# HiLab-git/WSL4MIS

Hardware: AMD Instinct MI355X
Metric: training slices/sec (256x256, bs64, unet_cct pCE+GatedCRF) (higher is better)
Workload: dtype f32; 1 GPU; unet_cct pce_gatedcrf r=5, 256x256x1 4-class synthetic scribble slices, batch 64/GPU, SGD+poly LR; global_batch=64, parallelism=dp1, crf_radius=5, conv_precision=f32

## Files before the change

include/wsl_hip.h:

```cpp
#ifndef WSL_HIP_H
#define WSL_HIP_H
#include <stddef.h>
#include <stdint.h>

#ifdef __cplusplus
extern "C" {
#endif

#define WSL_OK 0
#define WSL_EINVAL (-1)
#define WSL_EUNSUPPORTED (-2)
#define WSL_EHIP (-3)
#define WSL_EWORKSPACE (-4)

#define WSL_LEAKY_SLOPE 0.01f

int wsl_version(void);
const char* wsl_last_error(void);
const char* wsl_build_info(void);

#define WSL_PROF_FAMILIES 20
typedef struct WslProfRow {
  char name[48];
  int64_t calls;
// ... 43 lines not shown
                          int64_t* num_batches_tracked, float* mean, float* invstd, float* scale, float* shift,
                          void* stream);
int wsl_bn_eval_affine(const float* gamma, const float* beta, const float* running_mean, const float* running_var,
                       float eps, int C, float* scale, float* shift, void* stream);
int wsl_src_materialize(const WslSrc* s, float* out, int64_t out_bs, int N, int H, int W, void* stream);
int wsl_pool2_fwd(const WslSrc* s, float* out, int N, int H, int W, void* stream);

int wsl_feat_grad_combine(const WslSrc* f, const float* ga, int64_t ga_bs, const float* gb, int64_t gb_bs,
                          const float* gb_cmask, const float* gp, float* g, int N, int H, int W, void* stream);

int wsl_bnact_bwd(const float* g, int64_t g_bs, const float* y, const float* mean, const float* invstd,
                  const float* gamma, const float* beta, const uint8_t* emask, float emask_scale, float* dy,
                  float* dgamma, float* dbeta, int N, int C, int H, int W, void* ws, size_t ws_bytes, void* stream);
size_t wsl_bnact_bwd_ws_bytes(int N, int C, int H, int W);

int wsl_conv2d_dgrad_bn(const WslSrc* dy, const float* w, float* g, int64_t g_bs, int N, int H, int W, int Co, int ks,
                        int wmode, const float* bn_y, const float* bn_st, const uint8_t* bn_emask, float bn_emask_scale,
                        float* bn_part, int* fused, void* stream);
int wsl_feat_grad_combine_blocks(int N, int H, int W);
int wsl_feat_grad_combine_bn(const WslSrc* f, const float* ga, int64_t ga_bs, const float* gb, int64_t gb_bs,
                             const float* gb_cmask, const float* gp, float* g, int N, int H, int W, const float* bn_mean,
                             const float* bn_invstd, float* bn_part, void* stream);
int wsl_bnact_bwd_finish(const float* g, int64_t g_bs, const float* y, const float* mean, const float* invstd,
                         const float* gamma, const float* beta, const uint8_t* emask, float emask_scale, float* dy,
                         float* dgamma, float* dbeta, int N, int C, int H, int W, const float* part, int nblk,
                         int channel_major, void* ws, size_t ws_bytes, void* stream);
int wsl_conv2d_dgrad_bn_d(const WslSrc* dy, const float* w, float* g, int64_t g_bs, int N, int H, int W, int Co, int ks,
                          int wmode, const float* bn_y, const float* bn_st, const uint8_t* bn_emask, float bn_emask_scale,
                          float* bn_part, int* fused, void* stream);
int wsl_bnact_bwd_finish_d_amax(const float* dz, int64_t dz_bs, const float* y, const float* mean, const float* invstd,
                                const float* gamma, const float* beta, float* dy, float* dgamma, float* dbeta, int N, int C, int H,
                                int W, const float* part, int nblk, int channel_major, void* ws, size_t ws_bytes, uint32_t* dy_amax,
                                void* stream);

#define WSL_SP_ACT_EXP 4
#define WSL_SP_AMAX_SLOTS 64
int wsl_sp_conv2d_ok(const WslSrc* a, const WslSrc* b, const float* y, int64_t y_bs, int N, int H, int W, int Co, int ks);
size_t wsl_sp_weight_image_bytes(int Co, int Ci);
int wsl_sp_pack_weights(const float* w, void* image, uint32_t* w_amax, int Co, int Ci, int dgrad, void* stream);
int wsl_sp_conv2d_fwd(const WslSrc* a, const WslSrc* b, const void* image, const uint32_t* w_amax, const uint32_t* in_amax,
                      const float* bias, float* y, int64_t y_bs, int N, int H, int W, int Co, float* stat_part, float* stat_cnt,
                      void* stream);
int wsl_sp_conv2d_stat_blocks(int N, int H, int W, int Ci, int Co);
int wsl_sp_conv2d_dgrad_bn(const WslSrc* dy, const uint32_t* dy_amax, const void* image, const uint32_t* w_amax, float* g,
                           int64_t g_bs, int N, int H, int W, int Co, const float* bn_y, const float* bn_st,
                           const uint8_t* bn_emask, float bn_emask_scale, float* bn_part, int* fused, void* stream);
size_t wsl_sp_conv2d_wgrad_ws_bytes(int N, int H, int W, int Ci, int Co);
int wsl_sp_conv2d_wgrad_partial(const WslSrc* a, const WslSrc* b, const float* dy, int64_t dy_bs, const uint32_t* dy_amax,
                                float* dw, float* db, int N, int H, int W, int Co, void* ws, size_t ws_bytes,
                                WslWgradPending* pending, void* stream);
size_t wsl_bilinear_up2_fwd_amax_ws_bytes(int N, int C, int h, int w);
int wsl_bilinear_up2_fwd_amax(const float* u, float* out, int64_t out_bs, int N, int C, int h, int w, void* ws, size_t ws_bytes,
                              uint32_t* amax_slots, void* stream);
int wsl_sp_conv2d_wgrad_partial_amax(const WslSrc* a, const WslSrc* b, const float* dy, int64_t dy_bs, const uint32_t* dy_amax,
                                     const uint32_t* in_amax, float* dw, float* db, int N, int H, int W, int Co, void* ws,
                                     size_t ws_bytes, WslWgradPending* pending, void* stream);
size_t wsl_bnact_bwd_finish_ws_bytes(int N, int C, int H, int W, int with_amax);
int wsl_bnact_bwd_amax(const float* g, int64_t g_bs, const float* y, const float* mean, const float* invstd, const float* gamma,
                       const float* beta, const uint8_t* emask, float emask_scale, float* dy, float* dgamma, float* dbeta, int N,
                       int C, int H, int W, void* ws, size_t ws_bytes, uint32_t* dy_amax, void* stream);
int wsl_bnact_bwd_finish_amax(const float* g, int64_t g_bs, const float* y, const float* mean, const float* invstd,
                              const float* gamma, const float* beta, const uint8_t* emask, float emask_scale, float* dy,
                              float* dgamma, float* dbeta, int N, int C, int H, int W, const float* part, int nblk,
                              int channel_major, void* ws, size_t ws_bytes, uint32_t* dy_amax, void* stream);

int wsl_bilinear_up2_fwd(const float* u, float* out, int64_t out_bs, int N, int C, int h, int w, void* stream);
// ... 221 lines not shown
```

wsl4mis_amd/_lib.py:

```python
import ctypes as C
import os

import torch

_HERE = os.path.dirname(os.path.abspath(__file__))
LIB_PATH = os.path.join(_HERE, "csrc", "libwslhip.so")

c_fp = C.c_void_p


class WslSrc(C.Structure):
    _fields_ = [("x", c_fp), ("bs", C.c_int64), ("C", C.c_int32), ("_pad0", C.c_int32), ("scale", c_fp),
                ("shift", c_fp), ("emask", c_fp), ("emask_scale", C.c_float), ("_pad1", C.c_float), ("cmask", c_fp)]


WSL_PROF_FAMILIES = 20


class WslProfRow(C.Structure):
    _fields_ = [("name", C.c_char * 48), ("calls", C.c_int64), ("ms", C.c_double), ("flops", C.c_double),
                ("bytes", C.c_double), ("issued_flops", C.c_double)]


class WslNetDesc(C.Structure):
# ... 48 lines not shown
PQ = C.POINTER(WslPNetDesc)
PDAN = C.POINTER(WslDanDesc)

_PROTOS = {
    "wsl_version": (i32, []),
    "wsl_last_error": (C.c_char_p, []),
    "wsl_build_info": (C.c_char_p, []),
    "wsl_prof_enable": (i32, [i32]),
    "wsl_prof_report": (i32, [C.POINTER(WslProfRow), i32]),
    "wsl_net_concurrent": (i32, [i32]),
    "wsl_conv2d_fwd": (i32, [PS, PS, c_fp, c_fp, c_fp, i64, i32, i32, i32, i32, i32, i32, c_fp, c_fp, c_fp]),
    "wsl_conv2d_stat_blocks": (i32, [i32, i32, i32, i32, i32, i32]),
    "wsl_conv2d_pack_weights": (i32, [c_fp, c_fp, i32, i32, i32, i32, c_fp]),
    "wsl_conv2d_fast_ok": (i32, [PS, PS, c_fp, i64, i32]),
    "wsl_conv2d_wino_ok": (i32, [i32, i32, i32, i32, i32, i32, i32]),
    "wsl_conv2d_wgrad": (i32, [PS, PS, c_fp, i64, c_fp, c_fp, i32, i32, i32, i32, i32, c_fp, sz, c_fp]),
    "wsl_conv2d_wgrad_ws_bytes": (sz, [i32, i32, i32, i32, i32, i32]),
    "wsl_conv2d_wgrad_partial": (i32, [PS, PS, c_fp, i64, c_fp, c_fp, i32, i32, i32, i32, i32, c_fp, sz,
                                       C.POINTER(WslWgradPending), c_fp]),
    "wsl_wgrad_reduce_batch": (i32, [C.POINTER(WslWgradPending), i32, c_fp]),
    "wsl_bn_stats_finalize": (i32, [c_fp, c_fp, i32, i32, c_fp, c_fp, f32, f32, c_fp, c_fp, c_fp, c_fp, c_fp, c_fp,
                                    c_fp, c_fp]),
    "wsl_bn_eval_affine": (i32, [c_fp, c_fp, c_fp, c_fp, f32, i32, c_fp, c_fp, c_fp]),
    "wsl_src_materialize": (i32, [PS, c_fp, i64, i32, i32, i32, c_fp]),
    "wsl_pool2_fwd": (i32, [PS, c_fp, i32, i32, i32, c_fp]),
    "wsl_feat_grad_combine": (i32, [PS, c_fp, i64, c_fp, i64, c_fp, c_fp, c_fp, i32, i32, i32, c_fp]),
    "wsl_bnact_bwd": (i32, [c_fp, i64, c_fp, c_fp, c_fp, c_fp, c_fp, c_fp, f32, c_fp, c_fp, c_fp, i32, i32, i32, i32,
                            c_fp, sz, c_fp]),
    "wsl_bnact_bwd_ws_bytes": (sz, [i32, i32, i32, i32]),
    "wsl_conv2d_dgrad_bn": (i32, [PS, c_fp, c_fp, i64, i32, i32, i32, i32, i32, i32, c_fp, c_fp, c_fp, f32, c_fp, C.POINTER(C.c_int), c_fp]),
    "wsl_conv2d_dgrad_bn_d": (i32, [PS, c_fp, c_fp, i64, i32, i32, i32, i32, i32, i32, c_fp, c_fp, c_fp, f32, c_fp, C.POINTER(C.c_int), c_fp]),
    "wsl_bnact_bwd_finish_d_amax": (i32, [c_fp, i64, c_fp, c_fp, c_fp, c_fp, c_fp, c_fp, c_fp, c_fp, i32, i32, i32, i32,
                                          c_fp, i32, i32, c_fp, sz, c_fp, c_fp]),
    "wsl_feat_grad_combine_blocks": (i32, [i32, i32, i32]),
    "wsl_feat_grad_combine_bn": (i32, [PS, c_fp, i64, c_fp, i64, c_fp, c_fp, c_fp, i32, i32, i32, c_fp, c_fp, c_fp, c_fp]),
    "wsl_bnact_bwd_finish": (i32, [c_fp, i64, c_fp, c_fp, c_fp, c_fp, c_fp, c_fp, f32, c_fp, c_fp, c_fp, i32, i32, i32, i32,
                                   c_fp, i32, i32, c_fp, sz, c_fp]),
    "wsl_sp_conv2d_ok": (i32, [PS, PS, c_fp, i64, i32, i32, i32, i32, i32]),
    "wsl_sp_weight_image_bytes": (sz, [i32, i32]),
    "wsl_sp_pack_weights": (i32, [c_fp, c_fp, c_fp, i32, i32, i32, c_fp]),
    "wsl_sp_conv2d_fwd": (i32, [PS, PS, c_fp, c_fp, c_fp, c_fp, c_fp, i64, i32, i32, i32, i32, c_fp, c_fp, c_fp]),
    "wsl_sp_conv2d_stat_blocks": (i32, [i32, i32, i32, i32, i32]),
    "wsl_sp_conv2d_dgrad_bn": (i32, [PS, c_fp, c_fp, c_fp, c_fp, i64, i32, i32, i32, i32, c_fp, c_fp, c_fp, f32, c_fp,
                                     C.POINTER(C.c_int), c_fp]),
    "wsl_sp_conv2d_wgrad_ws_bytes": (sz, [i32, i32, i32, i32, i32]),
    "wsl_sp_conv2d_wgrad_partial": (i32, [PS, PS, c_fp, i64, c_fp, c_fp, c_fp, i32, i32, i32, i32, c_fp, sz,
                                          C.POINTER(WslWgradPending), c_fp]),
    "wsl_sp_conv2d_wgrad_partial_amax": (i32, [PS, PS, c_fp, i64, c_fp, c_fp, c_fp, c_fp, i32, i32, i32, i32, c_fp, sz,
                                               C.POINTER(WslWgradPending), c_fp]),
    "wsl_bilinear_up2_fwd_amax_ws_bytes": (sz, [i32, i32, i32, i32]),
    "wsl_bilinear_up2_fwd_amax": (i32, [c_fp, c_fp, i64, i32, i32, i32, i32, c_fp, sz, c_fp, c_fp]),
    "wsl_bnact_bwd_finish_ws_bytes": (sz, [i32, i32, i32, i32, i32]),
    "wsl_bnact_bwd_amax": (i32, [c_fp, i64, c_fp, c_fp, c_fp, c_fp, c_fp, c_fp, f32, c_fp, c_fp, c_fp, i32, i32, i32, i32,
                                 c_fp, sz, c_fp, c_fp]),
    "wsl_bnact_bwd_finish_amax": (i32, [c_fp, i64, c_fp, c_fp, c_fp, c_fp, c_fp, c_fp, f32, c_fp, c_fp, c_fp, i32, i32, i32, i32,
                                        c_fp, i32, i32, c_fp, sz, c_fp, c_fp]),
    "wsl_bilinear_up2_fwd": (i32, [c_fp, c_fp, i64, i32, i32, i32, i32, c_fp]),
    "wsl_bilinear_up2_bwd": (i32, [c_fp, i64, c_fp, i32, i32, i32, i32, c_fp]),
    "wsl_softmax_fwd": (i32, [c_fp, c_fp, i32, i32, i32, c_fp]),
    "wsl_softmax_bwd": (i32, [c_fp, c_fp, c_fp, i32, i32, i32, c_fp]),
    "wsl_ce_fwd_bwd": (i32, [c_fp, c_fp, i32, i32, c_fp, c_fp, f32, i32, i32, i32, c_fp, sz, c_fp]),
    "wsl_mix_argmax": (i32, [c_fp, c_fp, f64, c_fp, i32, i32, i32, c_fp]),
    "wsl_pdice_fwd": (i32, [c_fp, c_fp, i32, i32, c_fp, c_fp, i32, i32, i32, c_fp, sz, c_fp]),
    "wsl_pdice_bwd": (i32, [c_fp, c_fp, i32, i32, c_fp, c_fp, c_fp, i32, i32, i32, c_fp]),
    "wsl_head_fwd_bwd": (i32, [c_fp, c_fp, c_fp, i32, f64, f32, f32, c_fp, c_fp, c_fp, c_fp, i32, i32, i32, c_fp, sz,
                               c_fp]),
# ... 176 lines not shown
```

wsl4mis_amd/csrc/wsl_bn.hip:

```cpp
#include <stdlib.h>

#include "wsl_rt.h"

namespace wsl {

constexpr int kChunk = 4096;

constexpr int kFinalizeWideFrom = 2048;
static inline int finalize_threads(int nblk) { return nblk >= kFinalizeWideFrom ? 1024 : kThreads; }
template <int NV>
__device__ __forceinline__ void finalize_merge_waves(double (&v)[NV], double* red) {
  const int nw = blockDim.x >> 6, w = threadIdx.x >> 6;
#pragma unroll
  for (int m = 32; m >= 1; m >>= 1)
#pragma unroll
    for (int k = 0; k < NV; ++k) v[k] += __shfl_xor(v[k], m);
  if ((threadIdx.x & 63) == 0)
#pragma unroll
    for (int k = 0; k < NV; ++k) red[k * 16 + w] = v[k];
  __syncthreads();
#pragma unroll
  for (int k = 0; k < NV; ++k) {
    double t[16];
#pragma unroll
// ... 356 lines not shown
  const float sc = p.gamma[c] * invstd, sh = fmaf(-mean, sc, p.beta[c]);
  const float c1 = coef[2 * c], c2 = coef[2 * c + 1];
  const int base = blockIdx.x * kChunk;
  float m = 0.f;
  for (int i = base + 4 * threadIdx.x; i < base + kChunk && i < p.HW; i += 4 * kThreads) {
    float d[4], xh[4];
    bn_dz4(p, n, c, i, sc, sh, mean, invstd, d, xh);
    const float4 v = make_float4(sc * (d[0] - c1 - xh[0] * c2), sc * (d[1] - c1 - xh[1] * c2), sc * (d[2] - c1 - xh[2] * c2),
                                 sc * (d[3] - c1 - xh[3] * c2));
    *reinterpret_cast<float4*>(dy + ((int64_t)n * p.C + c) * p.HW + i) = v;
    if (pmax) m = fmaxf(fmaxf(m, fmaxf(fabsf(v.x), fabsf(v.y))), fmaxf(fabsf(v.z), fabsf(v.w)));
  }
  if (pmax) amax_block_store(m, pmax);
}

__global__ __launch_bounds__(1024) void bnact_bwd_finalize_kernel(const float* part, int nblk, int C, int64_t sb, int64_t sc,
                                                                  double count, float* dgamma, float* dbeta, float* coef) {
  __shared__ double red[2 * 16];
  const int c = blockIdx.x;
  double acc[2] = {0, 0};
#pragma unroll 8
  for (int b = threadIdx.x; b < nblk; b += blockDim.x) {
    const float2 v = *reinterpret_cast<const float2*>(part + ((int64_t)b * sb + (int64_t)c * sc) * 2);
    acc[0] += v.x;
    acc[1] += v.y;
  }
  finalize_merge_waves<2>(acc, red);
  const double s1 = acc[0], s2 = acc[1];
  if (threadIdx.x == 0) {
    if (dbeta) dbeta[c] = (float)s1;
    if (dgamma) dgamma[c] = (float)s2;
    coef[2 * c] = (float)(s1 / count);
    coef[2 * c + 1] = (float)(s2 / count);
  }
}

__global__ __launch_bounds__(256) void bnact_bwd_apply_kernel(BnBwdP p, const float* coef, float* dy, uint32_t* pmax) {
  const int c = blockIdx.y, n = blockIdx.z;
  const float mean = p.mean[c], invstd = p.invstd[c];
  const float sc = p.gamma[c] * invstd, sh = fmaf(-mean, sc, p.beta[c]);
  const float c1 = coef[2 * c], c2 = coef[2 * c + 1];
  const int base = blockIdx.x * kChunk;
  float m = 0.f;
  for (int i = base + threadIdx.x; i < base + kChunk && i < p.HW; i += kThreads) {
    float xh;
    const float d = bn_dz(p, n, c, i, sc, sh, mean, invstd, &xh);
    const float v = sc * (d - c1 - xh * c2);
    dy[((int64_t)n * p.C + c) * p.HW + i] = v;
    m = fmaxf(m, fabsf(v));
  }
  if (pmax) amax_block_store(m, pmax);
}

__device__ __forceinline__ void lerp_coord(int dst, float scale, int in, int* i0, int* i1, float* l) {
  const float src = scale * (float)dst;
  int a = (int)src;
  if (a > in - 1) a = in - 1;
  *i0 = a;
  *i1 = a + (a < in - 1 ? 1 : 0);
  *l = src - (float)a;
}

__global__ __launch_bounds__(256) void bilinear_up2_fwd_kernel(const float* u, float* out, int64_t out_bs, int C, int h,
                                                               int w) {
  const int c = blockIdx.y, n = blockIdx.z, Ho = 2 * h, Wo = 2 * w;
  const float sy = Ho > 1 ? (float)(h - 1) / (float)(Ho - 1) : 0.f, sx = Wo > 1 ? (float)(w - 1) / (float)(Wo - 1) : 0.f;
// ... 342 lines not shown
  p.g_is_d = g_is_d;
  ProfScope ps(PF_BN_BWD, 0.0, (double)N * C * H * W * (12.0 + (emask && !g_is_d ? 1.0 : 0.0)), stream);
  float* coef = static_cast<float*>(ws);
  dim3 grid(p.chunks, C, N);
  auto al16 = [](const void* q) { return (reinterpret_cast<uintptr_t>(q) & 15) == 0; };
  const bool vec = (H * W) % 4 == 0 && (g_bs % 4) == 0 && al16(g) && al16(y) && al16(dy) &&
                   (!emask || (reinterpret_cast<uintptr_t>(emask) & 3) == 0);
  WSL_LAUNCH(bnact_bwd_finalize_kernel, dim3(C), dim3(finalize_threads(nblk)), 0, stream, part, nblk, C,
             channel_major ? (int64_t)1 : (int64_t)C, channel_major ? (int64_t)nblk : (int64_t)1, (double)N * H * W, dgamma, dbeta,
             coef);
  uint32_t* pmax = dy_amax ? reinterpret_cast<uint32_t*>(coef + 2 * (size_t)C) : nullptr;
  if (vec) WSL_LAUNCH(bnact_bwd_apply4_kernel, grid, dim3(kThreads), 0, stream, p, coef, dy, pmax);
  else WSL_LAUNCH(bnact_bwd_apply_kernel, grid, dim3(kThreads), 0, stream, p, coef, dy, pmax);
  if (dy_amax) WSL_LAUNCH(amax_fold_kernel, dim3(WSL_SP_AMAX_SLOTS), dim3(kThreads), 0, stream, pmax, N * p.chunks * C, dy_amax);
  return check_launch("bnact_bwd_finish");
}

extern "C" int wsl_bnact_bwd_finish_amax(const float* g, int64_t g_bs, const float* y, const float* mean, const float* invstd,
                                         const float* gamma, const float* beta, const uint8_t* emask, float emask_scale, float* dy,
                                         float* dgamma, float* dbeta, int N, int C, int H, int W, const float* part, int nblk,
                                         int channel_major, void* ws, size_t ws_bytes, uint32_t* dy_amax, void* stream) {
  return bnact_bwd_finish_impl(g, g_bs, y, mean, invstd, gamma, beta, emask, emask_scale, dy, dgamma, dbeta, N, C, H, W, part, nblk,
                               channel_major, ws, ws_bytes, dy_amax, 0, stream);
}

extern "C" int wsl_bnact_bwd_finish_d_amax(const float* d, int64_t d_bs, const float* y, const float* mean, const float* invstd,
                                           const float* gamma, const float* beta, float* dy, float* dgamma, float* dbeta, int N, int C,
                                           int H, int W, const float* part, int nblk, int channel_major, void* ws, size_t ws_bytes,
                                           uint32_t* dy_amax, void* stream) {
  return bnact_bwd_finish_impl(d, d_bs, y, mean, invstd, gamma, beta, nullptr, 1.f, dy, dgamma, dbeta, N, C, H, W, part, nblk,
                               channel_major, ws, ws_bytes, dy_amax, 1, stream);
}

extern "C" int wsl_bnact_bwd_finish(const float* g, int64_t g_bs, const float* y, const float* mean, const float* invstd,
                                    const float* gamma, const float* beta, const uint8_t* emask, float emask_scale, float* dy,
                                    float* dgamma, float* dbeta, int N, int C, int H, int W, const float* part, int nblk,
                                    int channel_major, void* ws, size_t ws_bytes, void* stream) {
  return wsl_bnact_bwd_finish_amax(g, g_bs, y, mean, invstd, gamma, beta, emask, emask_scale, dy, dgamma, dbeta, N, C, H, W, part,
                                   nblk, channel_major, ws, ws_bytes, nullptr, stream);
}

extern "C" int wsl_feat_grad_combine_blocks(int N, int H, int W) {
  return N > 0 && H > 0 && W > 0 ? N * cdiv(((H + 1) / 2) * ((W + 1) / 2), kChunk) : 0;
}

extern "C" int wsl_feat_grad_combine_bn(const WslSrc* f, const float* ga, int64_t ga_bs, const float* gb, int64_t gb_bs,
                                        const float* gb_cmask, const float* gp, float* g, int N, int H, int W,
                                        const float* bn_mean, const float* bn_invstd, float* bn_part, void* stream) {
  WSL_REQUIRE(f && f->x && f->scale && f->shift && !f->emask && !f->cmask && g && N > 0 && H > 0 && W > 0 && f->C > 0,
              "feat_grad_combine_bn: the feature must be a plain BatchNorm + LeakyReLU source");
  WSL_REQUIRE(bn_mean && bn_invstd && bn_part, "feat_grad_combine_bn: null BatchNorm argument");
  ProfScope ps(PF_POOL_FANIN, 0.0, (double)N * f->C * H * W * (4.0 * (ga ? 1 : 0) + 4.0 * (gb ? 1 : 0) + (gp ? 1.0 : 0.0) + 8.0), stream);
  WSL_LAUNCH(feat_grad_combine_bn_kernel, dim3(cdiv(((H + 1) / 2) * ((W + 1) / 2), kChunk), f->C, N), dim3(kThreads), 0,
             stream, *f, ga, ga_bs, gb, gb_bs, gb_cmask, gp, g, H, W, bn_mean, bn_invstd, bn_part);
  return check_launch("feat_grad_combine_bn_kernel");
}

extern "C" size_t wsl_bilinear_up2_fwd_amax_ws_bytes(int N, int C, int h, int w) {
  return N > 0 && C > 0 && h > 0 && w > 0 ? sizeof(uint32_t) * (size_t)N * C * cdiv(2 * h, kUpFR) : 0;
}

extern "C" int wsl_bilinear_up2_fwd_amax(const float* u, float* out, int64_t out_bs, int N, int C, int h, int w, void* ws, size_t ws_bytes,
                                         uint32_t* amax_slots, void* stream) {
  WSL_REQUIRE(u && out && N > 0 && C > 0 && h > 0 && w > 0, "bilinear_up2_fwd: bad args");
  WSL_REQUIRE(out_bs >= (int64_t)C * 4 * h * w, "bilinear_up2_fwd: out batch stride too small");
  if (amax_slots && (!ws || ws_bytes < wsl_bilinear_up2_fwd_amax_ws_bytes(N, C, h, w))) {
// ... 55 lines not shown
```

wsl4mis_amd/csrc/wsl_net.hip:

```cpp
#include <initializer_list>

#include "wsl_seq.h"

namespace wsl {

int sp_pack_table(const PackTable& t, const int64_t* img_off_bytes, const float* params, void* imgf, void* imgd, uint32_t* amax,
                  int with_dgrad, void* stream);

static const int kFt[5] = {16, 32, 64, 128, 256};
static const float kDrop[5] = {0.05f, 0.1f, 0.2f, 0.3f, 0.5f};
constexpr int kSpMaxLayers = 40;

struct BlockRef { ConvRef c1, c2; BnRef b1, b2; };
struct BlkWs { size_t y1, y2, st1, st2; };

struct Plan {
  WslNetDesc d;
  int H[5], W[5];
  BlockRef enc[5];
  struct Dec { ConvRef c1x1[4]; BlockRef blk[4]; ConvRef out; } dec[2];
  int64_t n_param, n_enc_param, n_buf, n_bn;
  BlkWs wenc[5];
  size_t pooled[5];
  struct DecWs { size_t u[4], up[4], dcat[4], glow4; BlkWs blk[4]; } wdec[2];
  struct Scratch { size_t tmp_g, tmp_g1, tmp_dy, tmp_du, tmp_gpool, stat_part, stat_cnt, wg_ws, bn_ws, bn_coef; } scr[2];
  size_t packf, packd;
  size_t winof, winod;
  size_t spf, spd, sp_wmax, sp_dymax, sp_upmax;
  int sp;
  size_t wg_bytes, bn_bytes, bn_coef_bytes, total_floats;
  struct Region { char name[48]; size_t off, n; } regs[192];
  int nregs;
  bool want_regions = false, regs_overflow = false;
};

static void plan_block(BlockRef& k, int Ci, int Co, int64_t& po, int64_t& bo, int64_t& nbn) {
  plan_conv(k.c1, Ci, Co, 3, po);
  plan_bn(k.b1, Co, po, bo, nbn);
  plan_conv(k.c2, Co, Co, 3, po);
  plan_bn(k.b2, Co, po, bo, nbn);
// ... 234 lines not shown
  }
  const float* w = c.params + cv.w;
  int wmode = 1;
  if (wsl_conv2d_fast_ok(&dys, nullptr, g, g_bs, W)) {
    if (wsl_conv2d_wino_ok(N, H, W, cv.Co, 0, Cg, cv.ks)) w = c.ws + c.P.winod + 2 * cv.w, wmode = 5;
    else w = c.ws + c.P.packd + cv.w, wmode = 3;
  }
  int fused = 0;
  WSL_TRY(wsl_conv2d_dgrad_bn_d(&dys, w, g, g_bs, N, H, W, Cg, cv.ks, wmode, c.ws + y, c.ws + st, emask, es, c.ws + c.S().bn_ws,
                                &fused, c.stream));
  gs->nblk = fused ? wsl_conv2d_stat_blocks(N, H, W, cv.Co, Cg, cv.ks) : 0;
  gs->channel_major = 1;
  gs->g_is_d = fused == 2;
  return WSL_OK;
}

static int bn_bwd(const Ctx& c, const float* g, int64_t g_bs, size_t y, size_t st, const BnRef& bn, const uint8_t* emask, float es,
                  float* dy, int H, int W, const GStats& gs) {
  const Plan& P = c.P;
  const int C = bn.C;
  const float* s = c.ws + st;
  if (gs.nblk && gs.g_is_d)
    return wsl_bnact_bwd_finish_d_amax(g, g_bs, c.ws + y, s, s + C, c.params + bn.gamma, c.params + bn.beta, dy, c.grads + bn.gamma,
                                       c.grads + bn.beta, P.d.N, C, H, W, c.ws + c.S().bn_ws, gs.nblk, gs.channel_major,
                                       c.ws + c.S().bn_coef, P.bn_coef_bytes, sp_dymax(c, bn), c.stream);
  if (gs.nblk)
    return wsl_bnact_bwd_finish_amax(g, g_bs, c.ws + y, s, s + C, c.params + bn.gamma, c.params + bn.beta, emask, es, dy,
                                     c.grads + bn.gamma, c.grads + bn.beta, P.d.N, C, H, W, c.ws + c.S().bn_ws, gs.nblk,
                                     gs.channel_major, c.ws + c.S().bn_coef, P.bn_coef_bytes, sp_dymax(c, bn), c.stream);
  return wsl_bnact_bwd_amax(g, g_bs, c.ws + y, s, s + C, c.params + bn.gamma, c.params + bn.beta, emask, es, dy, c.grads + bn.gamma,
                            c.grads + bn.beta, P.d.N, C, H, W, c.ws + c.S().bn_ws, P.bn_bytes, sp_dymax(c, bn), c.stream);
}

static int pack_all(const Ctx& c, int with_dgrad) {
  const Plan& P = c.P;
  PackTable t;
  t.n = 0;
  auto one = [&](const ConvRef& cv, int l, int ca = 0, int cb = 0) {
    int skip = 0;
    if (cv.ks == 3) {
      const int N = P.d.N, H = P.H[l], W = P.W[l];
      if (wsl_conv2d_wino_ok(N, H, W, ca ? ca : cv.Ci, cb, cv.Co, 3)) skip |= 1;
      if (wsl_conv2d_wino_ok(N, H, W, cv.Co, 0, cv.Ci, 3)) skip |= 2;
    }
    t.e[t.n++] = PackEntry{cv.w, cv.Co, cv.Ci, cv.ks * cv.ks, skip};
  };
  for (int l = 0; l < 5; ++l) one(P.enc[l].c1, l), one(P.enc[l].c2, l);
  for (int k = 0; k < P.d.n_dec; ++k) {
    for (int i = 0; i < 4; ++i) {
      const int l = 3 - i;
      one(P.dec[k].c1x1[i], l + 1), one(P.dec[k].blk[i].c1, l, kFt[l], kFt[l]), one(P.dec[k].blk[i].c2, l);
    }
    one(P.dec[k].out, 0);
  }
  WSL_TRY(conv2_pack_table(t, c.params, c.ws + P.packf, c.ws + P.packd, with_dgrad, c.stream));
  WSL_TRY(wino_pack_table(t, c.params, c.ws + P.winof, c.ws + P.winod, with_dgrad, c.stream));
  if (P.sp) {
    WSL_REQUIRE(t.n <= kSpMaxLayers, "net: %d conv layers exceed the split path's table (%d)", t.n, kSpMaxLayers);
    int64_t off[kSpMaxLayers];
    for (int i = 0; i < t.n; ++i) off[i] = 4 * (int64_t)(4 * ((10 * t.e[i].w + 35) / 36));
    if (hipMemsetAsync(c.ws + P.sp_wmax, 0, kSpMaxLayers * sizeof(float), (hipStream_t)c.stream) != hipSuccess ||
        (with_dgrad && hipMemsetAsync(c.ws + P.sp_dymax, 0, (size_t)P.n_bn * WSL_SP_AMAX_SLOTS * sizeof(float), (hipStream_t)c.stream) != hipSuccess)) {
      set_error("net: clearing the split path's maxima failed");
      return WSL_EHIP;
    }
    WSL_TRY(sp_pack_table(t, off, c.params, c.ws + P.spf, c.ws + P.spd, reinterpret_cast<uint32_t*>(c.ws + P.sp_wmax), with_dgrad,
// ... 7 lines not shown
  const Plan& P = c.P;
  const int N = P.d.N, C = cv.Co;
  float* stp = c.training ? c.ws + c.S().stat_part : nullptr;
  float* stc = c.training ? c.ws + c.S().stat_cnt : nullptr;
  WSL_TRY(conv_any(c, cv, 0, a, b, c.params + cv.b, c.ws + y, (int64_t)C * H * W, H, W, stp, stc, raw_amax));
  float* s = c.ws + st;
  const int nblk = !c.training ? 0
                   : sp_takes(c, cv, a, b, c.ws + y, (int64_t)C * H * W, H, W, C) ? wsl_sp_conv2d_stat_blocks(N, H, W, cv.Ci, C)
                                                                                  : wsl_conv2d_stat_blocks(N, H, W, cv.Ci, C, cv.ks);
  return bn_fwd(c.training, stp, stc, nblk, bn, c.params, c.buffers, c.nbt, s, s + C, s + 2 * C, s + 3 * C, c.stream);
}

static int block_fwd(const Ctx& c, const BlockRef& k, const BlkWs& w, const WslSrc* a, const WslSrc* b, int l,
                     const uint8_t* emask, float es, const uint32_t* raw_amax = nullptr) {
  const int H = c.P.H[l], W = c.P.W[l], C = k.c1.Co;
  WSL_TRY(conv_bn_fwd(c, k.c1, k.b1, a, b, w.y1, w.st1, H, W, raw_amax));
  const WslSrc mid = act_src(c, w.y1, w.st1, C, H * W, c.training ? emask : nullptr, es, nullptr);
  return conv_bn_fwd(c, k.c2, k.b2, &mid, nullptr, w.y2, w.st2, H, W);
}

static int block_bwd(const Ctx& c, const BlockRef& k, const BlkWs& w, const WslSrc* a, const WslSrc* b, int l,
                     const uint8_t* emask, float es, const float* g, int64_t g_bs, const GStats& gs, float* dgrad_out,
                     const uint32_t* raw_amax = nullptr) {
  const Plan& P = c.P;
  const int H = P.H[l], W = P.W[l], C = k.c1.Co;
  const int64_t CHW = (int64_t)C * H * W;
  float* dy = c.ws + c.S().tmp_dy;
  float* g1 = c.ws + c.S().tmp_g1;
  WSL_TRY(bn_bwd(c, g, g_bs, w.y2, w.st2, k.b2, nullptr, 1.f, dy, H, W, gs));
  const WslSrc mid = act_src(c, w.y1, w.st1, C, H * W, emask, es, nullptr);
  WSL_TRY(wgrad_layer(c, &mid, nullptr, dy, CHW, c.grads + k.c2.w, c.grads + k.c2.b, H, W, C, 3, sp_dymax(c, k.b2)));
  GStats g1s;
  WSL_TRY(conv_dgrad_bn(c, k.c2, dy, g1, H, W, w.y1, w.st1, emask, es, &g1s, sp_dymax(c, k.b2)));
  WSL_TRY(bn_bwd(c, g1, CHW, w.y1, w.st1, k.b1, emask, es, dy, H, W, g1s));
  WSL_TRY(wgrad_layer(c, a, b, dy, CHW, c.grads + k.c1.w, c.grads + k.c1.b, H, W, C, 3, sp_dymax(c, k.b1), raw_amax));
  if (dgrad_out) {
    const WslSrc dys1 = raw_src(dy, C, CHW);
    WSL_TRY(conv_any(c, k.c1, 1, &dys1, nullptr, nullptr, dgrad_out, (int64_t)k.c1.Ci * H * W, H, W, nullptr, nullptr,
                     sp_dymax(c, k.b1)));
  }
  return WSL_OK;
}

static WslSrc feat_src(const Ctx& c, int l, const float* cmask) {
  return act_src(c, c.P.wenc[l].y2, c.P.wenc[l].st2, kFt[l], c.P.H[l] * c.P.W[l], nullptr, 1.f, cmask);
}

static int decoder_fwd(const Ctx& c, int k, const float* const* cmasks, float* logits) {
  const Plan& P = c.P;
  const int N = P.d.N;
  for (int i = 0; i < 4; ++i) {
    const int l = 3 - i, c1 = kFt[l + 1], c2 = kFt[l];
    const int h = P.H[l + 1], w = P.W[l + 1], H = P.H[l], W = P.W[l];
    const WslSrc low = i == 0 ? feat_src(c, 4, cmasks ? cmasks[4] : nullptr)
                              : act_src(c, P.wdec[k].blk[i - 1].y2, P.wdec[k].blk[i - 1].st2, c1, h * w, nullptr, 1.f, nullptr);
    const ConvRef& cv = P.dec[k].c1x1[i];
    WSL_TRY(conv_any(c, cv, 0, &low, nullptr, c.params + cv.b, c.ws + P.wdec[k].u[i], (int64_t)c2 * h * w, h, w, nullptr,
                     nullptr));
    WSL_TRY(wsl_bilinear_up2_fwd_amax(c.ws + P.wdec[k].u[i], c.ws + P.wdec[k].up[i], (int64_t)c2 * H * W, N, c2, h, w,
                                      c.ws + c.S().bn_coef, P.bn_coef_bytes, sp_upmax(c, k, i), c.stream));
    const WslSrc skip = feat_src(c, l, cmasks ? cmasks[l] : nullptr);
    const WslSrc up = raw_src(c.ws + P.wdec[k].up[i], c2, (int64_t)c2 * H * W);
    WSL_TRY(block_fwd(c, P.dec[k].blk[i], P.wdec[k].blk[i], &skip, &up, l, nullptr, 1.f, sp_upmax(c, k, i)));
  }
  const WslSrc last = act_src(c, P.wdec[k].blk[3].y2, P.wdec[k].blk[3].st2, kFt[0], P.H[0] * P.W[0], nullptr, 1.f, nullptr);
  const ConvRef& oc = P.dec[k].out;
// ... 381 lines not shown
```

Baseline: 4148 slices/s.

## Fuse first-conv BN backward finish with its weight-gradient partials

Adds a kernel that applies the BN/activation backward finish on the fly and accumulates the 3x3 weight and bias gradient partials for the very first encoder conv (1 input channel, 16 outputs). This skips writing the dy tensor and re-reading it in a separate wgrad kernel for the largest-resolution layer. The kernel double-buffers input tiles in shared memory and does a split reduction into pending partials. It drops emask handling for this path, and it is gated to cases with no dgrad output, W divisible by 64, and a raw unscaled input.

```diff
diff --git a/include/wsl_hip.h b/include/wsl_hip.h
--- a/include/wsl_hip.h
+++ b/include/wsl_hip.h
@@ -99,6 +99,10 @@
                                 const float* gamma, const float* beta, float* dy, float* dgamma, float* dbeta, int N, int C, int H,
                                 int W, const float* part, int nblk, int channel_major, void* ws, size_t ws_bytes, uint32_t* dy_amax,
                                 void* stream);
+int wsl_bnact_bwd_finish_d_wgrad_partial(const float* dz, int64_t dz_bs, const float* y, const float* mean, const float* invstd,
+                                         const float* gamma, const WslSrc* in, float* dgamma, float* dbeta, float* dw, float* db,
+                                         int N, int C, int H, int W, const float* part, int nblk, int channel_major, void* ws,
+                                         size_t ws_bytes, void* wg_ws, size_t wg_ws_bytes, WslWgradPending* pending, void* stream);
 
 #define WSL_SP_ACT_EXP 4
 #define WSL_SP_AMAX_SLOTS 64
diff --git a/wsl4mis_amd/_lib.py b/wsl4mis_amd/_lib.py
--- a/wsl4mis_amd/_lib.py
+++ b/wsl4mis_amd/_lib.py
@@ -104,6 +104,8 @@
     "wsl_conv2d_dgrad_bn_d": (i32, [PS, c_fp, c_fp, i64, i32, i32, i32, i32, i32, i32, c_fp, c_fp, c_fp, f32, c_fp, C.POINTER(C.c_int), c_fp]),
     "wsl_bnact_bwd_finish_d_amax": (i32, [c_fp, i64, c_fp, c_fp, c_fp, c_fp, c_fp, c_fp, c_fp, c_fp, i32, i32, i32, i32,
                                           c_fp, i32, i32, c_fp, sz, c_fp, c_fp]),
+    "wsl_bnact_bwd_finish_d_wgrad_partial": (i32, [c_fp, i64, c_fp, c_fp, c_fp, c_fp, PS, c_fp, c_fp, c_fp, c_fp, i32, i32, i32, i32,
+                                                   c_fp, i32, i32, c_fp, sz, c_fp, sz, C.POINTER(WslWgradPending), c_fp]),
     "wsl_feat_grad_combine_blocks": (i32, [i32, i32, i32]),
     "wsl_feat_grad_combine_bn": (i32, [PS, c_fp, i64, c_fp, i64, c_fp, c_fp, c_fp, i32, i32, i32, c_fp, c_fp, c_fp, c_fp]),
     "wsl_bnact_bwd_finish": (i32, [c_fp, i64, c_fp, c_fp, c_fp, c_fp, c_fp, c_fp, f32, c_fp, c_fp, c_fp, i32, i32, i32, i32,
diff --git a/wsl4mis_amd/csrc/wsl_bn.hip b/wsl4mis_amd/csrc/wsl_bn.hip
--- a/wsl4mis_amd/csrc/wsl_bn.hip
+++ b/wsl4mis_amd/csrc/wsl_bn.hip
@@ -412,6 +412,168 @@
     if (dgamma) dgamma[c] = (float)s2;
     coef[2 * c] = (float)(s1 / count);
     coef[2 * c + 1] = (float)(s2 / count);
+  }
+}
+
+struct BnWgP {
+  const float* d;
+  int64_t d_bs;
+  const float* y;
+  const float* mean;
+  const float* invstd;
+  const float* gamma;
+  const float* coef;
+  const float* x;
+  int64_t x_bs;
+  float* part_dw;
+  float* part_db;
+  int N, H, W, tiles_x, tiles_y, items, nsplit;
+};
+
+template <int CIN, int TW_>
+struct BnWgCfg {
+  static constexpr int TW = TW_, TH = TW == 64 ? 8 : 16;
+  static constexpr int XW = TW / 4, RG = 16 / XW, RPT = TH / RG;
+  static constexpr int ROWP = TW + 8, ROWS = TH + 2, ROWP4 = ROWP / 4, PB = ROWS * ROWP4, PLB = ROWS * ROWP;
+  static constexpr int NBF4 = CIN * PB, NB = (NBF4 + 255) / 256;
+  static constexpr int NACC = 9 * CIN + 1, RSTR = NACC | 1;
+  static_assert(TW == 64 || TW == 16, "tile widths built");
+};
+
+template <int CIN, int TW>
+__global__ __launch_bounds__(256, 3) void bnact_bwd_wgrad_small_kernel(BnWgP p) {
+  using C = BnWgCfg<CIN, TW>;
+  __shared__ __attribute__((aligned(16))) float xs[2][CIN * C::PLB];
+  __shared__ float red[kThreads * C::RSTR];
+  const int tid = threadIdx.x, c = tid >> 4, j = tid & 15;
+  const int x4 = j % C::XW, r0 = (j / C::XW) * C::RPT;
+  const bool interleaved = (p.nsplit & 7) == 0;
+  const int split = interleaved ? ((int)blockIdx.x & 7) * (p.nsplit >> 3) + ((int)blockIdx.x >> 3) : (int)blockIdx.x;
+  const int H = p.H, W = p.W, HW = H * W;
+  const float mean = p.mean[c], invstd = p.invstd[c];
+  const float sc = p.gamma[c] * invstd;
+  const float c1 = p.coef[2 * c], c2 = p.coef[2 * c + 1];
+
+  int bch[C::NB], brow[C::NB], bcol[C::NB], bl[C::NB];
+  bool bown[C::NB];
+#pragma unroll
+  for (int i = 0; i < C::NB; ++i) {
+    const int e = tid + i * kThreads;
+    bown[i] = e < C::NBF4;
+    const int ee = bown[i] ? e : 0;
+    bch[i] = ee / C::PB;
+    const int pos = ee - bch[i] * C::PB;
+    brow[i] = pos / C::ROWP4, bcol[i] = (pos - brow[i] * C::ROWP4) * 4;
+    bl[i] = bch[i] * C::PLB + brow[i] * C::ROWP + bcol[i];
+  }
+
+  const int it0 = interleaved ? split : (int)((int64_t)split * p.items / p.nsplit);
+  const int it_count = interleaved ? (p.items - split + p.nsplit - 1) / p.nsplit : (int)((int64_t)(split + 1) * p.items / p.nsplit) - it0;
+  const int step = interleaved ? p.nsplit : 1;
+  int nx_tx, nx_ty, nx_n;
+  {
+    int q = it0;
+    nx_tx = q % p.tiles_x;
+    q /= p.tiles_x;
+    nx_ty = q % p.tiles_y;
+    nx_n = q / p.tiles_y;
+  }
+  const int st_tx = step % p.tiles_x, st_ty = (step / p.tiles_x) % p.tiles_y, st_n = step / (p.tiles_x * p.tiles_y);
+  float4 prb[C::NB];
+  bool prok[C::NB];
+  int in_n = 0, in_y0 = 0, in_x0 = 0;
+  auto issue = [&]() __attribute__((always_inline)) {
+    in_n = nx_n, in_y0 = nx_ty * C::TH, in_x0 = nx_tx * C::TW;
+    nx_tx += st_tx;
+    const int cx = nx_tx >= p.tiles_x ? 1 : 0;
+    nx_tx -= cx ? p.tiles_x : 0;
+    nx_ty += st_ty + cx;
+    const int cy = nx_ty >= p.tiles_y ? 1 : 0;
+    nx_ty -= cy ? p.tiles_y : 0;
+    nx_n += st_n + cy;
+    const float* xb = p.x + in_n * p.x_bs;
+#pragma unroll
+    for (int i = 0; i < C::NB; ++i) {
+      const int gy = in_y0 + brow[i] - 1, gx = in_x0 + bcol[i] - 4;
+      prok[i] = bown[i] && gy >= 0 && gy < H && gx >= 0 && gx < W;
+      const uint32_t off = prok[i] ? (uint32_t)(bch[i] * HW + gy * W + gx) : 0u;
+      prb[i] = *reinterpret_cast<const float4*>(xb + off);
+    }
+  };
+
+  float acc[C::NACC];
+#pragma unroll
+  for (int k = 0; k < C::NACC; ++k) acc[k] = 0.f;
+
+  if (it_count > 0) issue();
+  for (int item = 0; item < it_count; ++item) {
+    float* xt = xs[item & 1];
+#pragma unroll
+    for (int i = 0; i < C::NB; ++i)
+      if (bown[i]) *reinterpret_cast<float4*>(xt + bl[i]) = prok[i] ? prb[i] : make_float4(0.f, 0.f, 0.f, 0.f);
+    const int n = in_n, y0 = in_y0, x0 = in_x0;
+    __syncthreads();
+    if (item + 1 < it_count) issue();
+
+    const int gx = x0 + 4 * x4;
+    const float* db_ = p.d + n * p.d_bs + (int64_t)c * HW;
+    const float* yb_ = p.y + ((int64_t)n * 16 + c) * HW;
+    float4 dv[C::RPT], yv[C::RPT];
+    bool ok[C::RPT];
+#pragma unroll
+    for (int rr = 0; rr < C::RPT; ++rr) {
+      const int gy = y0 + r0 + rr;
+      ok[rr] = gx < W && gy < H;
+      const uint32_t off = ok[rr] ? (uint32_t)(gy * W + gx) : 0u;
+      dv[rr] = *reinterpret_cast<const float4*>(db_ + off);
+      yv[rr] = *reinterpret_cast<const float4*>(yb_ + off);
+    }
+    float xw[CIN][3][6];
+    auto read6 = [&](int ci, int hrow, float (&dst)[6]) __attribute__((always_inline)) {
+      const float* b = xt + ci * C::PLB + hrow * C::ROWP + 4 * x4;
+      const float4 m = *reinterpret_cast<const float4*>(b + 4);
+      dst[0] = b[3], dst[1] = m.x, dst[2] = m.y, dst[3] = m.z, dst[4] = m.w, dst[5] = b[8];
+    };
+#pragma unroll
+    for (int ci = 0; ci < CIN; ++ci) read6(ci, r0, xw[ci][1]), read6(ci, r0 + 1, xw[ci][2]);
+#pragma unroll
+    for (int rr = 0; rr < C::RPT; ++rr) {
+#pragma unroll
+      for (int ci = 0; ci < CIN; ++ci) {
+#pragma unroll
+        for (int k = 0; k < 6; ++k) xw[ci][0][k] = xw[ci][1][k], xw[ci][1][k] = xw[ci][2][k];
+        read6(ci, r0 + rr + 2, xw[ci][2]);
+      }
+      const float d4[4] = {dv[rr].x, dv[rr].y, dv[rr].z, dv[rr].w}, y4[4] = {yv[rr].x, yv[rr].y, yv[rr].z, yv[rr].w};
+#pragma unroll
+      for (int e = 0; e < 4; ++e) {
+        const float xh = (y4[e] - mean) * invstd;
+        float v = sc * (d4[e] - c1 - xh * c2);
+        v = ok[rr] ? v : 0.f;
+        acc[9 * CIN] += v;
+#pragma unroll
+        for (int ci = 0; ci < CIN; ++ci)
+#pragma unroll
+          for (int ky = 0; ky < 3; ++ky)
+#pragma unroll
+            for (int kx = 0; kx < 3; ++kx) acc[ci * 9 + ky * 3 + kx] = fmaf(v, xw[ci][ky][e + kx], acc[ci * 9 + ky * 3 + kx]);
+      }
+    }
+  }
+
+#pragma unroll
+  for (int k = 0; k < C::NACC; ++k) red[tid * C::RSTR + k] = acc[k];
+  __syncthreads();
+  for (int o = tid; o < 16 * C::NACC; o += kThreads) {
+    const int co = o / C::NACC, k = o - co * C::NACC;
+    float sum = 0.f;
+    for (int jj = 0; jj < 16; ++jj) sum += red[(co * 16 + jj) * C::RSTR + k];
+    if (k < 9 * CIN) {
+      const int ci = k / 9, tap = k - ci * 9;
+      p.part_dw[(((int64_t)split * 9 + tap) * 16 + co) * CIN + ci] = sum;
+    } else {
+      p.part_db[(int64_t)split * 16 + co] = sum;
+    }
   }
 }
 
@@ -820,6 +982,69 @@
                                channel_major, ws, ws_bytes, dy_amax, 1, stream);
 }
 
+namespace wsl {
+bool bnact_bwd_wgrad_ok(const WslSrc& in, const float* dz, int64_t dz_bs, const float* y, int C, int H, int W) {
+  auto al16 = [](const void* q) { return (reinterpret_cast<uintptr_t>(q) & 15) == 0; };
+  if (C != 16 || in.C != 1 || in.scale || in.emask || in.cmask || H <= 0 || W <= 0 || (W & 3)) return false;
+  if (!al16(in.x) || !al16(dz) || !al16(y) || (in.bs & 3) || (dz_bs & 3)) return false;
+  return (int64_t)16 * H * W < (int64_t(1) << 31) && in.bs >= (int64_t)H * W && dz_bs >= (int64_t)16 * H * W;
+}
+}
+
+template <int CIN, int TW>
+static int launch_bnact_bwd_wgrad(BnWgP& p, void* stream) {
+  using K = BnWgCfg<CIN, TW>;
+  p.tiles_x = cdiv(p.W, K::TW), p.tiles_y = cdiv(p.H, K::TH);
+  WSL_LAUNCH((bnact_bwd_wgrad_small_kernel<CIN, TW>), dim3(p.nsplit), dim3(kThreads), 0, stream, p);
+  return check_launch("bnact_bwd_wgrad_small_kernel");
+}
+
+extern "C" int wsl_bnact_bwd_finish_d_wgrad_partial(const float* dz, int64_t dz_bs, const float* y, const float* mean, const float* invstd,
+                                                    const float* gamma, const WslSrc* in, float* dgamma, float* dbeta, float* dw,
+                                                    float* db, int N, int C, int H, int W, const float* part, int nblk,
+                                                    int channel_major, void* ws, size_t ws_bytes, void* wg_ws, size_t wg_ws_bytes,
+                                                    WslWgradPending* pending, void* stream) {
+  WSL_REQUIRE(dz && y && mean && invstd && gamma && in && dw && db && ws && wg_ws && part && pending,
+              "bnact_bwd_finish_d_wgrad: null argument");
+  WSL_REQUIRE(N > 0 && nblk > 0, "bnact_bwd_finish_d_wgrad: bad shape");
+  if (!bnact_bwd_wgrad_ok(*in, dz, dz_bs, y, C, H, W)) {
+    set_error("bnact_bwd_finish_d_wgrad: built for one raw input channel, 16 output channels, W %% 4 == 0 and 16-byte aligned tensors");
+    return WSL_EUNSUPPORTED;
+  }
+  if (ws_bytes < wsl_bnact_bwd_finish_ws_bytes(N, C, H, W, 0)) {
+    set_error("bnact_bwd_finish_d_wgrad: workspace %zu < %zu", ws_bytes, wsl_bnact_bwd_finish_ws_bytes(N, C, H, W, 0));
+    return WSL_EWORKSPACE;
+  }
+  constexpr int CIN = 1;
+  BnWgP p;
+  p.d = dz, p.d_bs = dz_bs, p.y = y, p.mean = mean, p.invstd = invstd, p.gamma = gamma, p.x = in->x, p.x_bs = in->bs;
+  p.N = N, p.H = H, p.W = W;
+  const bool wide = W % 64 == 0;
+  p.items = wide ? N * cdiv(H, BnWgCfg<CIN, 64>::TH) * (W / 64) : N * cdiv(H, BnWgCfg<CIN, 16>::TH) * cdiv(W, 16);
+  const size_t per_split = sizeof(float) * (9 * 16 * CIN + 16);
+  const int want = forced_wgrad_wgs() > 0 ? forced_wgrad_wgs() : 768;
+  int64_t ns = p.items < want ? p.items : want;
+  const int64_t fit = (int64_t)(wg_ws_bytes / per_split);
+  if (ns > fit) ns = fit >= 8 ? fit & ~(int64_t)7 : fit;
+  if (ns < 1) {
+    set_error("bnact_bwd_finish_d_wgrad: partials workspace %zu < %zu", wg_ws_bytes, per_split);
+    return WSL_EWORKSPACE;
+  }
+  p.nsplit = (int)ns;
+  p.part_dw = static_cast<float*>(wg_ws), p.part_db = p.part_dw + (size_t)p.nsplit * 9 * 16 * CIN;
+  float* coef = static_cast<float*>(ws);
+  p.coef = coef;
+  const double px = (double)N * H * W;
+  ProfScope ps(PF_BN_BWD, 2.0 * px * 16 * CIN * 9, 4.0 * px * (2 * 16 + CIN), stream);
+  WSL_LAUNCH(bnact_bwd_finalize_kernel, dim3(C), dim3(finalize_threads(nblk)), 0, stream, part, nblk, C,
+             channel_major ? (int64_t)1 : (int64_t)C, channel_major ? (int64_t)nblk : (int64_t)1, (double)N * H * W, dgamma, dbeta,
+             coef);
+  if (int rc = wide ? launch_bnact_bwd_wgrad<CIN, 64>(p, stream) : launch_bnact_bwd_wgrad<CIN, 16>(p, stream)) return rc;
+  pending->part_dw = p.part_dw, pending->part_db = p.part_db, pending->dw = dw, pending->db = db;
+  pending->Co = 16, pending->Ci = CIN, pending->KK = 9, pending->nsplit = p.nsplit;
+  return WSL_OK;
+}
+
 extern "C" int wsl_bnact_bwd_finish(const float* g, int64_t g_bs, const float* y, const float* mean, const float* invstd,
                                     const float* gamma, const float* beta, const uint8_t* emask, float emask_scale, float* dy,
                                     float* dgamma, float* dbeta, int N, int C, int H, int W, const float* part, int nblk,
diff --git a/wsl4mis_amd/csrc/wsl_net.hip b/wsl4mis_amd/csrc/wsl_net.hip
--- a/wsl4mis_amd/csrc/wsl_net.hip
+++ b/wsl4mis_amd/csrc/wsl_net.hip
@@ -6,6 +6,7 @@
 
 int sp_pack_table(const PackTable& t, const int64_t* img_off_bytes, const float* params, void* imgf, void* imgd, uint32_t* amax,
                   int with_dgrad, void* stream);
+bool bnact_bwd_wgrad_ok(const WslSrc& in, const float* dz, int64_t dz_bs, const float* y, int C, int H, int W);
 
 static const int kFt[5] = {16, 32, 64, 128, 256};
 static const float kDrop[5] = {0.05f, 0.1f, 0.2f, 0.3f, 0.5f};
@@ -306,6 +307,28 @@
                             c.grads + bn.beta, P.d.N, C, H, W, c.ws + c.S().bn_ws, P.bn_bytes, sp_dymax(c, bn), c.stream);
 }
 
+#ifndef WSL_FIRST_CONV_FUSED
+#define WSL_FIRST_CONV_FUSED 1
+#endif
+static bool bn_bwd_wgrad_takes(const Ctx& c, const ConvRef& cv, const WslSrc* a, const WslSrc* b, const float* d, int64_t d_bs, size_t y,
+                               int H, int W, const GStats& gs) {
+  if (WSL_TUNE("WSL_FIRST_CONV_FUSED", WSL_FIRST_CONV_FUSED) == 0) return false;
+  if (W % 64) return false;
+  return !b && cv.ks == 3 && gs.nblk && gs.g_is_d && bnact_bwd_wgrad_ok(*a, d, d_bs, c.ws + y, cv.Co, H, W);
+}
+static int bn_bwd_wgrad(const Ctx& c, const ConvRef& cv, const WslSrc* a, const float* d, int64_t d_bs, size_t y, size_t st,
+                        const BnRef& bn, int H, int W, const GStats& gs) {
+  const Plan& P = c.P;
+  const float* s = c.ws + st;
+  const size_t need = (wsl_conv2d_wgrad_ws_bytes(P.d.N, H, W, cv.Ci, cv.Co, 3) + 255) & ~(size_t)255;
+  return wgrad_push(c.wb, "net", c.ws + c.S().wg_ws, need, [&](void* ws, size_t n, WslWgradPending* q) {
+    return wsl_bnact_bwd_finish_d_wgrad_partial(d, d_bs, c.ws + y, s, s + bn.C, c.params + bn.gamma, a, c.grads + bn.gamma,
+                                                c.grads + bn.beta, c.grads + cv.w, c.grads + cv.b, P.d.N, bn.C, H, W,
+                                                c.ws + c.S().bn_ws, gs.nblk, gs.channel_major, c.ws + c.S().bn_coef, P.bn_coef_bytes, ws, n,
+                                                q, c.stream);
+  });
+}
+
 static int pack_all(const Ctx& c, int with_dgrad) {
   const Plan& P = c.P;
   PackTable t;
@@ -379,6 +402,8 @@
   WSL_TRY(wgrad_layer(c, &mid, nullptr, dy, CHW, c.grads + k.c2.w, c.grads + k.c2.b, H, W, C, 3, sp_dymax(c, k.b2)));
   GStats g1s;
   WSL_TRY(conv_dgrad_bn(c, k.c2, dy, g1, H, W, w.y1, w.st1, emask, es, &g1s, sp_dymax(c, k.b2)));
+  if (!dgrad_out && bn_bwd_wgrad_takes(c, k.c1, a, b, g1, CHW, w.y1, H, W, g1s))
+    return bn_bwd_wgrad(c, k.c1, a, g1, CHW, w.y1, w.st1, k.b1, H, W, g1s);
   WSL_TRY(bn_bwd(c, g1, CHW, w.y1, w.st1, k.b1, emask, es, dy, H, W, g1s));
   WSL_TRY(wgrad_layer(c, a, b, dy, CHW, c.grads + k.c1.w, c.grads + k.c1.b, H, W, C, 3, sp_dymax(c, k.b1), raw_amax));
   if (dgrad_out) {
```

Result: no change. 4182 slices/s (median of 6 runs) (+0.8%).
